# PaddlePaddle/Anakin

Hardware: AMD Instinct MI355X
Metric: ResNet50 INT8 images/sec + p50 latency @ batch 1/8, 1×MI355X (higher is better)
Workload: dtype int8

## Files before the change

### anakin_amd/csrc/api_chain.hip

```cpp
#include "api_internal.h"

enum : unsigned { CK_1X1 = 1, CK_3X3 = 2, CK_HEAD = 4, CK_PAIR = 8, CK_LED = CK_3X3 | CK_HEAD, CK_ANY = 15 };
static unsigned chain_kind(const saber_hip_chain* ch) { return !ch->c3 ? CK_1X1 : (ch->b2 ? CK_PAIR : (ch->b ? CK_3X3 : CK_HEAD)); }
static const struct { int c1; unsigned kinds; ChainForm f; } chain_forms[] = {
    {64, CK_ANY,            {4, 4, 4, 1, 1, CS_BASE, false}},
    {64, CK_ANY,            {2, 2, 4, 1, 1, CS_BASE, false}},
    {128, CK_1X1 | CK_LED,  {2, 2, 4, 1, 1, CS_BASE, false}},
    {128, CK_1X1 | CK_LED,  {1, 1, 4, 1, 1, CS_BASE, false}},
    {128, CK_1X1 | CK_LED,  {6, 2, 8, 1, 1, CS_W8, false}},
    {128, CK_1X1 | CK_LED,  {5, 1, 8, 1, 1, CS_W8, false}},
    {256, CK_1X1 | CK_LED,  {1, 1, 4, 1, 1, CS_BASE, false}},
    {256, CK_1X1,           {9, 1, 4, 2, 1, CS_SPLIT, false}},
    {256, CK_1X1,           {11, 1, 8, 2, 1, CS_SPLIT8, false}},
    {256, CK_LED,           {3, 1, 8, 1, 1, CS_W8, false}},
    {256, CK_3X3,           {7, 1, 8, 1, 2, CS_COOP2, true}},
    {256, CK_3X3,           {15, 2, 8, 1, 4, CS_COOP4, true}},
    {512, CK_1X1,           {1, 1, 4, 1, 1, CS_BASE, false}},
    {512, CK_1X1,           {9, 1, 4, 2, 1, CS_SPLIT, false}},
};
static void for_each_chain_form(const saber_hip_chain* ch, const std::function<void(const ChainForm&)>& fn) {
    for (const auto& r : chain_forms)
        if (r.c1 == ch->c1 && (r.kinds & chain_kind(ch))) fn(r.f);
}
static ChainForm chain_form_where(const saber_hip_chain* ch, const std::function<bool(const ChainForm& row, const ChainForm& found)>& take) {
// ... 159 lines not shown
    hipError_t e = sp->d_w.upload(w);
    if (e == hipSuccess) e = sp->d_prm.upload(prm);
    if (e != hipSuccess) {
        delete sp;
        return hip_fail(e, "stem pair: device copies");
    }
    *out = sp;
    return SABER_HIP_OK;
}
void saber_hip_conv2d_stem_pair_destroy(saber_hip_stem_pair_t* sp) { delete sp; }
int saber_hip_conv2d_stem_pair_run(saber_hip_stem_pair_t* sp, const void* x, void* y_pool, void* y_a, void* y_b, void* workspace,
                                   saber_hip_stream_t stream) {
    if (g_capture) return capture_unsupported("saber_hip_conv2d_stem_pair_run (an executor-level object: saber_hip_net_optimize forms it itself)");
    if (!sp || !x || !y_a || !y_b) return fail(SABER_HIP_INVALID_VALUE, "null argument");
    saber_hip_conv* op = sp->stem;
    if (op->ws_bytes && !workspace) return fail(SABER_HIP_INVALID_VALUE, "workspace required");
    saber_mi355x::StemPairKArgs ka;
    const int rc = stem_pool_args(op, x, y_pool, workspace, (hipStream_t)stream, &ka.c);
    if (rc) return rc;
    ka.t.w = sp->d_w.p; ka.t.prm = sp->d_prm.p; ka.t.y1 = y_a; ka.t.y2 = y_b;
    ka.t.K1 = sp->a->d.k; ka.t.K2 = sp->b->d.k;
    ka.t.relu1 = sp->a->d.act == SABER_HIP_ACT_RELU; ka.t.relu2 = sp->b->d.act == SABER_HIP_ACT_RELU;
    ka.t.u8_1 = sp->a->d.out_dtype == SABER_HIP_U8; ka.t.u8_2 = sp->b->d.out_dtype == SABER_HIP_U8;
    HIP_TRY(saber_mi355x::launch_conv_stem_pool_pair(op->pre_quant ? 1 : 0, ka, (hipStream_t)stream));
    return SABER_HIP_OK;
}
saber_hip_chain::~saber_hip_chain() {
    if (h_coop_err) (void)hipHostFree(h_coop_err);
    delete stage1;
}
static unsigned div_magic(int d) { return d >= 2 ? (unsigned)((0x100000000ull + (unsigned)d - 1) / (unsigned)d) : 0u; }
static int stage_build(saber_hip_chain* const* chains, int n, bool per_image, saber_hip_chain* tail, saber_hip_chain_stage** out,
                       const saber_hip_conv* head_a = nullptr, const saber_hip_conv* head_b = nullptr) {
    if (!chains || n <= 0 || n > saber_mi355x::STAGE4_LONG || !out) return fail(SABER_HIP_INVALID_VALUE, "stage: 1..24 chains");
    if (head_a || head_b) {
        if (!head_a || !head_b) return fail(SABER_HIP_INVALID_VALUE, "null argument");
        if (!chains[0] || chains[0]->c1 != 256) return fail(SABER_HIP_INVALID_VALUE, "stage: a head goes with a C = 256 stage only");
        if (!per_image) return fail(SABER_HIP_INVALID_VALUE, "stage: a head needs an image per XCD");
        for (const saber_hip_conv* o : {head_a, head_b})
            if (o->d.res_mode != SABER_HIP_RES_NONE) return fail(SABER_HIP_INVALID_VALUE, "stage: the head's convs carry no residual");
        for (const saber_hip_conv* o : {head_a, head_b}) {
            const saber_hip_conv_desc& d = o->d;
            if (!o->is_i8 || !o->weights_set || o->algo != ALGO_IGEMM_I8 || o->epi != EPI_I8_CONV || o->pair_k2 || o->pool_fused || o->pool2 || o->gpool ||
                o->pre_quant || o->pre_pad || d.kh != 1 || d.kw != 1 || d.stride_h != 1 || d.stride_w != 1 || d.pad_h != 0 || d.pad_w != 0 || d.group != 1 ||
                o->c_eff != d.c || d.act_negative_slope != 0.f || d.in_layout != SABER_HIP_NHWC || d.out_layout != SABER_HIP_NHWC ||
                (d.out_dtype != SABER_HIP_S8 && d.out_dtype != SABER_HIP_U8))
                return fail(SABER_HIP_INVALID_VALUE, "stage: the head must be two plain 1x1 / stride 1 / pad 0 INT8 NHWC convs with weights set");
// ... 405 lines not shown
```

### anakin_amd/csrc/api_conv.hip

```cpp
#include "api_internal.h"

namespace saber_api {
thread_local std::string g_err;

void* zero_page() {
    static std::mutex mu;
    static void* pages[64] = {nullptr};
    int dev = 0;
    if (hipGetDevice(&dev) != hipSuccess || dev < 0 || dev >= 64) return nullptr;
    std::lock_guard<std::mutex> lock(mu);
    if (!pages[dev]) {
        void* p = nullptr;
        if (hipMalloc(&p, 256) != hipSuccess) return nullptr;
        if (hipMemset(p, 0, 256) != hipSuccess || hipStreamSynchronize(nullptr) != hipSuccess) {
            (void)hipFree(p);
            return nullptr;
        }
        pages[dev] = p;
    }
    return pages[dev];
}

}

// ... 608 lines not shown

int saber_hip_conv2d_run(saber_hip_conv_t* op, const void* x, void* y, const void* res, void* workspace,
                         saber_hip_stream_t stream) {
    if (g_capture) return capture_conv(op, x, y, res);
    if (!op || !x || !y) return fail(SABER_HIP_INVALID_VALUE, "null argument");
    if (!op->weights_set) return fail(SABER_HIP_INVALID_VALUE, "set_weights not called");
    if (op->ws_bytes && !workspace) return fail(SABER_HIP_INVALID_VALUE, "workspace required");
    if (op->d.res_mode == SABER_HIP_RES_ELTWISE && !res) return fail(SABER_HIP_INVALID_VALUE, "residual tensor required");
    if (op->pair_k2) return fail(SABER_HIP_INVALID_VALUE, "sibling pair: use saber_hip_conv2d_run_pair");
    hipStream_t s = (hipStream_t)stream;
    const saber_hip_conv_desc& d = op->d;
    const void* xin = x;
    if (op->gpool) return fail(SABER_HIP_INVALID_VALUE, "conv + fused global pooling: use saber_hip_conv2d_run_gpool");
    if (op->sel.fam == FAM_IMG1) return img_conv_run(op, x, y, res, nullptr, s);
    if (op->stem32) {
        HIP_TRY(launch_conv_stem_f32_pool_raw((const float*)x, op->d_wstem32.p, op->has_bias ? op->d_bias.p : nullptr, (float*)y, d.n, d.h, d.w, op->oh,
                                              op->ow, op->pool_oh, op->pool_ow, op->stem32 - 1, s));
        return SABER_HIP_OK;
    }
    if (op->pool_fused) {
        ConvKArgs a;
        const int rc = stem_pool_args(op, x, y, workspace, s, &a);
        if (rc) return rc;
        HIP_TRY(launch_conv_stem_pool(op->pre_quant ? 1 : 0, a, s));
        return SABER_HIP_OK;
    }
    if (op->sel.fam == FAM_STEM && op->pre_quant) {
        ConvKArgs a;
        fill_args(op, a, x, y, res);
        a.Cin = d.c;
        a.qinv = 1.f / op->in_scale;
        HIP_TRY(launch_conv_stem(1, a, s));
        return SABER_HIP_OK;
    }
    if (op->pre_quant) {
        HIP_TRY(launch_quantize_nchw_to_nhwc(d.n, d.c, d.h, d.w, op->c_eff, DT_S8, op->in_scale, (const float*)x,
                                             workspace, s));
        xin = workspace;
    } else if (op->pre_pad) {
        HIP_TRY(launch_pad_channels_i8((size_t)d.n * d.h * d.w, d.c, 4, x, workspace, s));
        xin = workspace;
    } else if (op->pre_transpose) {
        HIP_TRY(launch_transpose_nchw_to_nhwc_f32(d.n, d.c, d.h, d.w, op->c_eff, (const float*)x, (float*)workspace, s));
        xin = workspace;
    }
    ConvKArgs a;
    fill_args(op, a, xin, y, res);
// ... 107 lines not shown
```

### anakin_amd/csrc/api_internal.h

```cpp
#pragma once
#include "../../include/saber_hip.h"
#include "kernels.h"

#include <cmath>
#include <cstdio>
#include <algorithm>
#include <cstdlib>
#include <cstring>
#include <functional>
#include <memory>
#include <mutex>
#include <string>
#include <utility>
#include <type_traits>
#include <vector>

using namespace saber_mi355x;

namespace saber_api {

extern thread_local std::string g_err;
inline int fail(int code, const std::string& msg) {
    g_err = msg;
    return code;
// ... 87 lines not shown
inline ConvSel sel_halo(const ConvSel& base, int rows) { return sel_family(base, FAM_HALO, rows); }
inline ConvSel sel_img(const ConvSel& base, int nw, int ib, int rb) {
    ConvSel s = sel_family(base, FAM_IMG);
    s.img_nw = nw; s.img_ib = ib; s.img_rb = rb;
    return s;
}
inline ConvSel sel_img1(const ConvSel& base) { return sel_family(base, FAM_IMG1); }
inline ConvSel sel_fc_small(const ConvSel& base) { return sel_family(base, FAM_FC_SMALL); }
inline ConvSel sel_b3h(ConvSel base, int variant) { base.dma = 0; return sel_family(base, FAM_B3H, variant); }
inline ConvSel sel_pw(ConvSel base, int variant) { base.dma = 0; return sel_family(base, FAM_PW, variant); }
inline ConvSel sel_dw(const ConvSel& base, int form) { return sel_family(base, FAM_DW, form); }
inline ConvSel sel_group(const ConvSel& base, int form) { return sel_family(base, FAM_GROUP, form); }

}
using namespace saber_api;

struct saber_hip_conv {
    saber_hip_conv_desc d;
    int oh = 0, ow = 0;
    int algo = ALGO_DIRECT_I8;
    ConvSel sel;
    int pool_fused = 0, pool_oh = 0, pool_ow = 0;
    int pool2 = 0;
    int stem32 = 0;
    DevBuf<uint8_t> d_wstem32;
    std::vector<float> w_stem_host;
    DevBuf<uint8_t> d_w3h1, d_w3h2;
    DevBuf<uint8_t> d_wpw;
    DevBuf<uint8_t> d_wdw;
    DevBuf<uint8_t> d_wg;
    DevBuf<float> d_fcpart;
    DevBuf<unsigned> d_fcctr;
    DevBuf<float> d_wfc;
    int gpool = 0;
    struct saber_hip_stage* img_stage = nullptr;
    bool no_placement = false;
    int epi = EPI_I8_CONV;
    bool is_i8 = false;
    int x_dtype = DT_S8;
    int c_eff = 0;
    bool pre_quant = false;
    bool pre_pad = false;
    bool pre_transpose = false;
    size_t ws_bytes = 0;
    int Kg = 0, Kg_pad = 0, kw_pad = 0;
    float in_scale = 1.f, out_scale = 1.f;
// ... 362 lines not shown
```

### anakin_amd/csrc/api_net_autotune.hip

```cpp
#include "api_internal.h"

static saber_hip_conv* net_op_conv(saber_hip_net* net, int index) {
    if (index < 0 || index >= (int)net->ops.size()) return nullptr;
    NetOp& o = net->ops[index];
    if (o.kind == OP_CONV || o.kind == OP_CONV_PAIR) return o.conv;
    if (o.kind == OP_FC || o.kind == OP_FC_Q) return o.fc ? o.fc->conv : nullptr;
    return nullptr;
}
int saber_hip_net_get_choice(saber_hip_net_t* net, int index) {
    saber_hip_conv* c = net_op_conv(net, index);
    int choice = (c && !c->pool_fused && (c->algo <= ALGO_IGEMM_F32 || dw_ok(c) || group_ok(c))) ? saber_hip_conv2d_get_tile(c) : 0;
    if (!c) return choice;
    const NetOp& o = net->ops[index];
    if (o.chain) choice |= (1 << 28) | ((o.chain_on ? o.chain->form.code : 0) << 24);
    if (o.chain3) choice |= (1 << 29) | ((o.led_on ? o.chain3->form.code : 0) << 24);
    if (o.sep) choice |= (3 << 28) | ((o.sep_on ? o.sep->form : 0) << 24);
    if (o.ir) choice |= (int)0x80000000u | ((o.ir_on ? o.ir->form : 0) << 24);
    if (o.fire) choice |= (int)0x80000000u | ((o.fire_on ? o.fire->form : 0) << 24);
    if (o.stage && o.stage_on) choice |= 1 << 30;
    if (o.stage && o.stage_on && o.tail_on) choice |= (int)0x80000000u;
    if (o.head_of >= 0 && net->ops[o.head_of].stage_on && net->ops[o.head_of].head_on) choice |= 1 << 29;
    return choice;
}
int saber_hip_net_stage_blocks(const saber_hip_net_t* net, int index) {
    if (!net || index < 0 || index >= (int)net->ops.size()) return 0;
    const NetOp& o = net->ops[index];
    return o.stage ? (o.stage->c1 == 64 ? -o.stage_n : o.stage_n) : 0;
}
int saber_hip_net_stage_head(const saber_hip_net_t* net, int index) {
    if (!net || index < 1 || index >= (int)net->ops.size() || !net->ops[index].stage) return -1;
    return net->ops[index - 1].head_of == index ? index - 1 : -1;
}
int saber_hip_net_set_choice(saber_hip_net_t* net, int index, int choice) {
    saber_hip_conv* c = net_op_conv(net, index);
    const bool ir_bits = c && net->ops[index].ir && ((unsigned)choice >> 30) == 2u;
    const int ir_tn = (choice >> 24) & 15;
    if (ir_bits && ir_tn && !ir_form_valid(net->ops[index].ir, ir_tn)) return saber_hip_conv2d_ir_set_tile(net->ops[index].ir, ir_tn);
    const bool fire_bits = c && net->ops[index].fire && ((unsigned)choice >> 30) == 2u;
    if (fire_bits && ir_tn && !fire_form_valid(net->ops[index].fire, ir_tn)) return saber_hip_conv2d_fire_set_tile(net->ops[index].fire, ir_tn);
    if (fire_bits && !(choice & 0xffffff)) {
        net_set_fire(net, index, ir_tn);
        net_drop_graph(net);
        return SABER_HIP_OK;
    }
    if (ir_bits && !(choice & 0xffffff)) {
        net_set_ir(net, index, ir_tn);
        net_drop_graph(net);
        return SABER_HIP_OK;
    }
    if (!c || !choice || c->pool_fused || (c->algo > ALGO_IGEMM_F32 && !dw_ok(c) && !group_ok(c))) return SABER_HIP_OK;
    if (net->reproducible_fp32 && !c->is_i8) return SABER_HIP_OK;
    if (net->ops[index].kind == OP_CONV_PAIR && index > 0 && net->ops[index - 1].stem_pair) return SABER_HIP_OK;
    const int chain_bits = (choice >> 24) & 63;
    const bool stage_on = ((choice >> 30) & 1) && !net->shared_device;
    const bool tail_on = stage_on && (((unsigned)choice >> 31) & 1u);
    choice &= 0xffffff;
    if (net->shared_device && ((choice >> 16) & 0xff) == 11) choice &= ~(0xf << 12);
    NetOp& o = net->ops[index];
    saber_hip_chain* ch = index + 1 >= (int)net->ops.size() ? nullptr : ((o.chain3 && (chain_bits & 32)) ? o.chain3 : ((o.chain && (chain_bits & 16)) ? o.chain : nullptr));
    int tn = chain_bits & 15;
    if (ch && net->shared_device && chain_form(ch, tn).placement) tn = chain_form_plain(ch).code;
    if (ch && tn && !chain_form_valid(ch, tn)) return saber_hip_conv2d_chain_set_tile(ch, tn);
    const bool sep_bits = o.sep && (chain_bits & 48) == 48;
    if (sep_bits && tn && !sep_form_valid(o.sep, tn)) return saber_hip_conv2d_sep_set_tile(o.sep, tn);
    int rc = choice ? saber_hip_conv2d_set_tile(c, choice) : SABER_HIP_OK;
    if (rc) return rc;
    o.res_note.clear();
    o.stage_name_kept = false;
    if (ch && tn) (void)saber_hip_conv2d_chain_set_tile(ch, tn);
// ... 105 lines not shown
        if (o.kind == OP_CONV_PAIR) {
            int rc = saber_hip_conv2d_autotune_pair(o.conv, T(o.in), T(o.out), T(o.out2), stream, iters);
            if (rc) return rc;
            continue;
        }
        saber_hip_conv* c = o.kind == OP_CONV ? o.conv : ((o.kind == OP_FC || o.kind == OP_FC_Q) ? o.fc->conv : nullptr);
        if (!c) continue;
        const void* xin = T(o.in);
        if (o.kind == OP_FC && o.fc->pre_quant) {
            int rq = net_launch(net, o, (hipStream_t)stream);
            if (rq) return rq;
            xin = net->arena + net->ws_off;
        }
        int rc = saber_hip_conv2d_autotune(c, xin, T(o.out), T(o.in2), net->arena + net->ws_off, stream, iters);
        if (rc) return rc;
        o.res_note.clear();
    }
    net_resolve(net);
    const char* log_env = std::getenv("SABER_HIP_AUTOTUNE_LOG");
    const bool log_cands = g_cold && log_env && log_env[0] == '1';
    auto log_cand = [&](const saber_hip_conv* c, const std::string& name, float t) {
        if (log_cands) std::fprintf(stderr, "autotune [%dx%dx%d c%d k%d %dx%d] %-40s %8.2f us\n", c->d.n, c->d.h, c->d.w, c->d.c, c->d.k, c->d.kh, c->d.kw, name.c_str(), t);
    };
    for (size_t i = 0; i < net->ops.size(); ++i)
        if (net->ops[i].stage) net_set_stage(net, (int)i, false);
    for (size_t i = 0; i < net->ops.size(); ++i) {
        NetOp& A = net->ops[i];
        const int ia = (int)i;
        NetOp* H = (ia > 0 && net->ops[ia - 1].chain3) ? &net->ops[ia - 1] : nullptr;
        if (!A.chain && !H) continue;
        const int first = H ? ia - 1 : ia;
        const int last = (A.chain || (H && H->chain3->b2)) ? ia + 1 : ia;
        hipStream_t s = (hipStream_t)stream;
        auto run_all = [&]() -> int {
            int rc = 0;
            for (int k = first; k <= last; ++k) rc |= net_launch(net, net->ops[k], s);
            return rc;
        };
        auto timed = [&](float* t) { return time_enqueued(s, run_all, 20, t); };
        float best = 0.f;
        int best_mode = 0, best_tn = 0;
        net_set_chain_mode(net, ia, 0);
        int rc = timed(&best);
        if (rc) return rc;
        log_cand(A.conv, "separate", best);
        for (int mode = A.chain ? 1 : 2; mode <= (H ? 2 : 1); ++mode) {
// ... 146 lines not shown
```

### anakin_amd/csrc/api_select.hip

```cpp
#include "api_internal.h"

bool dw_ok(const saber_hip_conv* op) {
    const saber_hip_conv_desc& d = op->d;
    if (op->algo != ALGO_DIRECT_I8 && op->algo != ALGO_DIRECT_F32) return false;
    if (d.res_mode != SABER_HIP_RES_NONE || op->pre_quant || op->pre_pad || op->pre_transpose || d.out_layout != SABER_HIP_NHWC) return false;
    if (op->is_i8 && op->epi != EPI_I8_CONV) return false;
    return conv_dw3x3_ok(!op->is_i8, d.n, d.c, d.k, d.group, d.kh, d.kw, d.stride_h, d.stride_w, d.pad_h, d.pad_w, d.dil_h, d.dil_w, op->oh, op->ow);
}
bool group_ok(const saber_hip_conv* op) {
    const saber_hip_conv_desc& d = op->d;
    if (op->algo != ALGO_DIRECT_I8 || !op->is_i8 || op->epi != EPI_I8_CONV) return false;
    if (d.res_mode != SABER_HIP_RES_NONE || op->pre_quant || op->pre_pad || d.in_layout != SABER_HIP_NHWC || d.out_layout != SABER_HIP_NHWC) return false;
    if (d.in_dtype != SABER_HIP_S8 && d.in_dtype != SABER_HIP_U8) return false;
    return conv_group3x3_ok(d.n, d.c, d.k, d.group, d.kh, d.kw, d.stride_h, d.stride_w, d.pad_h, d.pad_w, d.dil_h, d.dil_w, op->oh, op->ow);
}
static bool pw_variant_ok(const saber_hip_conv* op, int variant) {
    if (!pw_eligible(op)) return false;
    if (variant == 0) return conv1x1_pw_ok(op->c_eff, op->d.k);
    int tm, p, dd, mb;
    return conv1x1_pwk_variant(variant, &tm, &p, &dd, &mb) && conv1x1_pwk_ok(op->d.n * op->d.h * op->d.w, op->c_eff, op->d.k) &&
           (op->c_eff >> 7) >= dd;
}
bool b3_tile_ok(const saber_hip_conv* op, int tile, int ks) {
    if (op->algo != ALGO_IGEMM_F32 || !op->d_w3.p || tile < 0 || tile >= TILE_COUNT_B3 || (ks != 1 && ks != 2)) return false;
// ... 166 lines not shown
    case 10: *out = sel_fc_small(cur); return SABER_HIP_OK;
    case 11: *out = sel_b3(cur, low, (ks & 15) ? (ks & 15) : 1, ks >> 4); return SABER_HIP_OK;
    case 12: *out = sel_img1(cur); return SABER_HIP_OK;
    case 13: *out = sel_b3h(cur, low); return SABER_HIP_OK;
    case 14: *out = sel_pw(cur, low); return SABER_HIP_OK;
    case 16:
        if (!dw_ok(op) || low > DW3X3_FORMS) return fail(SABER_HIP_INVALID_VALUE, sel_requirements(FAM_DW));
        *out = low ? sel_dw(cur, low) : sel_direct(cur);
        return SABER_HIP_OK;
    case 17:
        if (!group_ok(op) || low > G3X3_FORMS) return fail(SABER_HIP_INVALID_VALUE, sel_requirements(FAM_GROUP));
        *out = low ? sel_group(cur, low) : sel_direct(cur);
        return SABER_HIP_OK;
    default: return fail(SABER_HIP_INVALID_VALUE, "bad staging variant");
    }
}

int saber_hip_conv2d_set_tile(saber_hip_conv_t* op, int tile) {
    if (op->stem32) {
        if (((tile >> 16) & 0xff) != 15 || (tile & 0xff) > 3) return fail(SABER_HIP_INVALID_VALUE, "FP32 stem launch: (15 << 16) | 0..3");
        op->stem32 = 1 + (tile & 0xff);
        return SABER_HIP_OK;
    }
    if (op->pool_fused) return fail(SABER_HIP_INVALID_VALUE, "fused conv+pooling has a single kernel");
    ConvSel s;
    const int rc = sel_decode(op, tile, &s);
    return rc ? rc : sel_set(op, s);
}
int saber_hip_conv2d_get_tile(const saber_hip_conv_t* op) { return sel_encode(op); }

void sel_name(saber_hip_conv* op) {
    static const char* an[] = {"igemm_i8", "igemm_i8_c4", "igemm_f32", "direct_i8", "direct_f32"};
    const ConvSel& s = op->sel;
    const saber_hip_conv_desc& d = op->d;
    const char* sum = d.res_mode == SABER_HIP_RES_SUM_INPLACE ? "+sum" : "";
    int bmk = 0, bnp = 0;
    int tm = 0, thr = 0, depth = 0, wgs = 0;
    char buf[96];
    if (op->stem32) snprintf(buf, sizeof buf, "stem7x7s2_maxpool3x3s2_f32_bf16x3_nchw_in");
    else if (op->pool_fused) snprintf(buf, sizeof buf, "stem7x7s2_maxpool3x3s2_i8_4x8%s", op->pre_quant ? "_fusedquant" : "");
    else switch (s.fam) {
    case FAM_STEM: snprintf(buf, sizeof buf, "stem7x7s2_i8_8x16%s", op->pre_quant ? "_fusedquant" : ""); break;
    case FAM_FC_SMALL:
        snprintf(buf, sizeof buf, op->algo == ALGO_IGEMM_F32 ? ((op->d_fcpart.p && !op->d_wfc.p) ? "fc_f32_splitk_16xk4" : "fc_f32_small_16xk4") : "fc_i8_small_16xk4");
        break;
    case FAM_PW:
        if (s.variant) {
            (void)conv1x1_pwk_variant(s.variant, &tm, &bnp, &depth, &wgs);
            snprintf(buf, sizeof buf, "pw1x1_f32_bf16x3_ksplit4_%dch_%dpx_d%d%s%s", tm * 16, bnp * 16, depth, wgs > 1 ? "_2wg" : "", sum);
        } else snprintf(buf, sizeof buf, "pw1x1_f32_bf16x3_regs_c%d_%dch_per_wave%s", op->c_eff, op->c_eff == 64 ? 64 : 32, sum);
        break;
    case FAM_B3H:
        (void)conv3x3_b3h_variant(s.variant, &bmk, &bnp, &tm, &thr);
        if (s.variant >= 6) snprintf(buf, sizeof buf, "pw1x1_f32_bf16x3_%dch_%dpx_w%d", bmk, bnp * 16, thr / 64);
        else snprintf(buf, sizeof buf, "halo3x3_f32_bf16x3_%dch_%dx16_w%d%s", bmk, bnp, thr / 64, op->pool2 ? "+maxpool2x2" : "");
        break;
    case FAM_IMG1: snprintf(buf, sizeof buf, "imgres%dx%d_i8_%dch%s", d.kh, d.kw, 16 * ((d.k / 16 + 31) / 32), op->gpool ? "+gpool" : ""); break;
    case FAM_IMG: snprintf(buf, sizeof buf, "img3x3_i8_%dimg_x_%drows_k16_w%d", s.img_ib, s.img_rb, s.img_nw); break;
    case FAM_HALO: snprintf(buf, sizeof buf, "halo3x3_i8_%dx16", s.variant); break;
    case FAM_DW: snprintf(buf, sizeof buf, "dw3x3_%s_%s", op->is_i8 ? "i8" : "f32", conv_dw3x3_form_name(s.variant, !op->is_i8)); break;
    case FAM_GROUP: snprintf(buf, sizeof buf, "g3x3_i8_%s", conv_group3x3_form_name(s.variant)); break;
    case FAM_DIRECT: snprintf(buf, sizeof buf, "%s", an[op->algo]); break;
    case FAM_B3:
// ... 151 lines not shown
```

### anakin_amd/csrc/conv_stem.h

```cpp
#pragma once
#include "epilogue_pack.h"

namespace saber_mi355x {

typedef int v2i __attribute__((ext_vector_type(2)));
typedef unsigned short us2_ __attribute__((ext_vector_type(2)));
__device__ __forceinline__ unsigned pk_max_u16_(unsigned a, unsigned b) {
    const us2_ r = __builtin_elementwise_max(__builtin_bit_cast(us2_, a), __builtin_bit_cast(us2_, b));
    return __builtin_bit_cast(unsigned, r);
}

template <bool F32IN, int NPIX, int ICP>
__device__ __forceinline__ void stage_input_patch(const ConvKArgs& a, int n, int iy0, int ix0, unsigned xmask, int tid,
                                                  unsigned* lds_x) {
    constexpr int NIT = (NPIX + 255) / 256;
    float fv[NIT][4];
    unsigned pv[NIT];
    bool ok[NIT];
    const size_t plane = (size_t)a.H * a.W;
#pragma unroll
    for (int it = 0; it < NIT; ++it) {
        const int idx = tid + it * 256;
        const int r = idx / ICP, c = idx - r * ICP;
        const int iy = iy0 + r, ix = ix0 + c;
        ok[it] = idx < NPIX && iy >= 0 && iy < a.H && ix >= 0 && ix < a.W;
        pv[it] = 0;
#pragma unroll
        for (int ch = 0; ch < 4; ++ch) fv[it][ch] = 0.f;
        if (ok[it]) {
            if constexpr (F32IN) {
                const float* xp = (const float*)a.x + ((size_t)n * a.Cin * a.H + iy) * a.W + ix;
#pragma unroll
                for (int ch = 0; ch < 4; ++ch)
                    if (ch < a.Cin) fv[it][ch] = xp[ch * plane];
            } else {
                pv[it] = ((const unsigned*)a.x)[((size_t)n * a.H + iy) * a.W + ix];
            }
        }
    }
#pragma unroll
    for (int it = 0; it < NIT; ++it) {
        const int idx = tid + it * 256;
        unsigned pk = pv[it];
        if constexpr (F32IN) {
            if (ok[it]) {
#pragma unroll
                for (int ch = 0; ch < 4; ++ch) {
                    if (ch < a.Cin) {
                        float v = __fmul_rn(fv[it][ch], a.qinv);
                        v = truncf(v + copysignf(0x1.fffffep-2f, v));
                        v = v < -128.f ? -128.f : (v > 127.f ? 127.f : v);
                        pk |= ((unsigned)((int)v) & 0xffu) << (8 * ch);
                    }
                }
            }
        }
        if (idx < NPIX) lds_x[idx] = pk ^ xmask;
    }
}

template <int EK, bool F32IN>
__global__ __launch_bounds__(256) void conv_stem7x7s2_kernel(const ConvKArgs a) {
    constexpr int TH = 8, TW = 16;
    constexpr int IR = (TH - 1) * 2 + 7 + 1;
    constexpr int ICP = 40;
// ... 295 lines not shown
            const int g = (wave + 4 * i) >> 1;
            if (g >= tng) break;
            const int kb = g * 32 + fq * 8;
            const v4i* pc = lds_tp + (kb >> 2) * 3;
            const v4i z = {0, 0, 0, 0};
            const v4i c0 = mma_step(taf[i][0], bfr, pc[2]), c1 = mma_step(taf[i][1], bfr, pc[5]);
            const bool second = kb >= t.K1;
            const bool ou8 = second ? t.u8_2 : t.u8_1;
            const float lo = (second ? t.relu2 : t.relu1) ? 0.f : -3.0e38f;
            const float off = ou8 ? 0.f : 128.f;
            const unsigned xm = ou8 ? 0u : 0x80808080u;
            const unsigned w0 = chain_out_pack(c0, z, __builtin_bit_cast(v4f, pc[1]), __builtin_bit_cast(v4f, pc[0]), lo, off, xm);
            const unsigned w1 = chain_out_pack(c1, z, __builtin_bit_cast(v4f, pc[4]), __builtin_bit_cast(v4f, pc[3]), lo, off, xm);
            if (tok) {
                uint8_t* y = second ? (uint8_t*)t.y2 + tpix * t.K2 + (kb - t.K1) : (uint8_t*)t.y1 + tpix * t.K1 + kb;
                *(uint2*)y = make_uint2(w0, w1);
            }
        }
        SABER_TL(6);
    }
    SABER_TL_FLUSH();
}

template <bool F32IN>
__global__ __launch_bounds__(256, 4) void conv_stem_pool_kernel(const ConvKArgs a) {
    conv_stem_pool_body<F32IN, false>(a, StemPairTail{});
}
template <bool F32IN>
__global__ __launch_bounds__(256, 4) void conv_stem_pool_pair_kernel(const StemPairKArgs ka) {
    conv_stem_pool_body<F32IN, true>(ka.c, ka.t);
}

static hipError_t launch_conv_stem_pool_inst(int f32_in, const ConvKArgs& a, hipStream_t s) {
    ConvKArgs b = a;
    b.npx = a.N * ((a.pool_ow + 7) / 8) * ((a.pool_oh + 3) / 4);
    b.nky = (a.K + 63) / 64;
    b.mg_npx = magic_div(b.npx, (long long)b.npx * b.nky);
    dim3 grid(b.npx * b.nky), block(256);
    if (f32_in) hipLaunchKernelGGL((conv_stem_pool_kernel<true>), grid, block, 0, s, b);
    else hipLaunchKernelGGL((conv_stem_pool_kernel<false>), grid, block, 0, s, b);
    return hipGetLastError();
}
static hipError_t launch_conv_stem_pool_pair_inst(int f32_in, const StemPairKArgs& ka, hipStream_t s) {
    StemPairKArgs b = ka;
    b.c.npx = ka.c.N * ((ka.c.pool_ow + 7) / 8) * ((ka.c.pool_oh + 3) / 4);
    b.c.nky = 1;
    b.c.mg_npx = magic_div(b.c.npx, (long long)b.c.npx);
    dim3 grid(b.c.npx), block(256);
    if (f32_in) hipLaunchKernelGGL((conv_stem_pool_pair_kernel<true>), grid, block, 0, s, b);
    else hipLaunchKernelGGL((conv_stem_pool_pair_kernel<false>), grid, block, 0, s, b);
    return hipGetLastError();
}

}
```

### anakin_amd/csrc/kernels.h

```cpp
#pragma once
#include <hip/hip_runtime.h>
#include <stddef.h>
#include <stdint.h>

#ifdef SABER_TIMELINE
extern __device__ unsigned long long* saber_tl_buf;
#define SABER_TL_DECL unsigned long long tl_[16] = {0, 0, 0, 0, 0, 0, 0, 0, 0, 0, 0, 0, 0, 0, 0, 0}
#define SABER_TL(i) tl_[i] = wall_clock64()
#define SABER_TL_FLUSH()                                                                   \
    do {                                                                                   \
        if (threadIdx.x == 0 && saber_tl_buf)                                              \
            for (int i_ = 0; i_ < 16; ++i_) saber_tl_buf[(size_t)blockIdx.x * 16 + i_] = tl_[i_]; \
    } while (0)
#else
#define SABER_TL_DECL do { } while (0)
#define SABER_TL(i) do { } while (0)
#define SABER_TL_FLUSH() do { } while (0)
#endif

namespace saber_mi355x {

enum { DT_F32 = 0, DT_S8 = 1, DT_U8 = 2 };

enum {
// ... 205 lines not shown
bool conv3x3_img_feasible(int C, int OW, int OH, int N, int nw, int ib, int rb);
bool conv3x3_b3h_variant(int variant, int* bmk, int* th, int* tm, int* threads);
bool conv1x1_pw_ok(int c, int k);
hipError_t launch_conv1x1_pw(const ConvKArgs& a, hipStream_t s);
bool conv1x1_pwk_variant(int v, int* tm, int* p, int* d, int* minb);
bool conv1x1_pwk_ok(int m, int c, int k);
hipError_t launch_conv1x1_pwk(int variant, const ConvKArgs& a, hipStream_t s);
hipError_t launch_conv3x3_b3h(int variant, const ConvKArgs& a, hipStream_t s);
hipError_t launch_fc_i8_small(const ConvKArgs& a, hipStream_t s);
bool fc_i8_small_ok(int m, int c, int kg_pad);
hipError_t launch_fc_f32_small(const ConvKArgs& a, bool packed, hipStream_t s);
int fc_f32_packed_steps(int c);
bool fc_f32_small_ok(int m, int c, int kg_pad);
bool fc_i8_small_softmax_ok(int m, int c, int kg_pad, int k);
hipError_t launch_fc_i8_small_softmax(const ConvKArgs& a, float* prob, unsigned* ctr, hipStream_t s);
bool fc_f32_splitk_ok(int m, int c, int kg_pad, int k, bool softmax);
size_t fc_f32_splitk_part_floats(int c, int k);
size_t fc_f32_splitk_counters(int k);
hipError_t launch_fc_f32_splitk(const ConvKArgs& a, float* part, unsigned* ctr, float* prob, hipStream_t s);
bool gemm_f32_rows_ok(int m, int k);
hipError_t launch_gemm_f32_rows(int m, int n, int k, float alpha, const float* A, const float* B, float beta, float* C, const void* zero,
                                hipStream_t s);
hipError_t launch_conv_stem(int f32_in, const ConvKArgs& a, hipStream_t s);
hipError_t launch_conv_stem_pool(int f32_in, const ConvKArgs& a, hipStream_t s);
hipError_t launch_conv_stem_pool_pair(int f32_in, const StemPairKArgs& a, hipStream_t s);
hipError_t launch_conv_direct(int is_f32, const ConvKArgs& a, int group, hipStream_t s);
constexpr int DW3X3_FORMS = 2;
const char* conv_dw3x3_form_name(int form, bool f32);
bool conv_dw3x3_ok(bool f32, int n, int c, int k, int group, int kh, int kw, int stride_h, int stride_w, int pad_h, int pad_w, int dil_h,
                   int dil_w, int oh, int ow);
hipError_t launch_conv_dw3x3(int form, bool f32, const ConvKArgs& a, hipStream_t s);
constexpr int G3X3_FORMS = 1;
const char* conv_group3x3_form_name(int form);
int conv_group3x3_steps(int cg);
bool conv_group3x3_ok(int n, int c, int k, int group, int kh, int kw, int stride_h, int stride_w, int pad_h, int pad_w, int dil_h, int dil_w,
                      int oh, int ow);
hipError_t launch_conv_group3x3(int form, const ConvKArgs& a, int group, hipStream_t s);

struct SepKArgs {
    const void* x;
    const void* wdw;
    const float* dw_bias;
    const float* dw_scale;
    const void* wpw;
    const void* prm;
    void* y_dw;
    void* y_pw;
    int N, H, W, C, OH, OW, K;
// ... 117 lines not shown
```

### anakin_amd/csrc/stem_pool.hip

```cpp
#include "conv_stem.h"
namespace saber_mi355x {
hipError_t launch_conv_stem_pool(int f32_in, const ConvKArgs& a, hipStream_t s) { return launch_conv_stem_pool_inst(f32_in, a, s); }
hipError_t launch_conv_stem_pool_pair(int f32_in, const StemPairKArgs& a, hipStream_t s) { return launch_conv_stem_pool_pair_inst(f32_in, a, s); }
}
```

### anakin_amd/saber.py

```python
import ctypes as C

import numpy as np
import torch

from . import lib as L

_TORCH_DT = {L.F32: torch.float32, L.S8: torch.int8, L.U8: torch.uint8}


def _stream():
    return C.c_void_p(torch.cuda.current_stream().cuda_stream)


def _p(t):
    return None if t is None else C.c_void_p(t.data_ptr())


def _np_ptr(a):
    return None if a is None else a.ctypes.data_as(C.c_void_p)


def dtype_code(t):
    return {torch.float32: L.F32, torch.int8: L.S8, torch.uint8: L.U8}[t.dtype]

# ... 83 lines not shown
        return self

    def out_shape(self):
        d = self.desc
        oh, ow = self.out_hw
        return (d.n, oh, ow, d.k) if d.out_layout == L.NHWC else (d.n, d.k, oh, ow)

    def new_output(self):
        return torch.empty(self.out_shape(), dtype=_TORCH_DT[self.desc.out_dtype], device="cuda")

    def dispatch(self, x, y, res=None):
        L.check(L.load().saber_hip_conv2d_run(self.h, _p(x), _p(y), _p(res), _p(self.ws), _stream()))
        if getattr(self, "post_act", None) is not None:
            active, slope, coef = self.post_act
            activation(active, y, y, slope, coef)
        return y

    def algo(self):
        return L.load().saber_hip_conv2d_algo(self.h).decode()

    def set_tile(self, tile):
        L.check(L.load().saber_hip_conv2d_set_tile(self.h, tile))

    def set_global_pooling(self):
        L.check(L.load().saber_hip_conv2d_set_global_pooling(self.h))
        return self

    def dispatch_gpool(self, x, y, y_pool, res=None):
        L.check(L.load().saber_hip_conv2d_run_gpool(self.h, _p(x), _p(y), _p(res), _p(y_pool), _stream()))
        return y, y_pool

    def tile_id(self):
        return L.load().saber_hip_conv2d_get_tile(self.h) & 0xff

    def autotune(self, x, y, res=None, iters=5):
        L.check(L.load().saber_hip_conv2d_autotune(self.h, _p(x), _p(y), _p(res), _p(self.ws), _stream(), iters))

    def quantized_weights(self):
        d = self.desc
        wq = np.empty((d.k, d.c // d.group, d.kh, d.kw), np.int8)
        ws = np.empty(d.k, np.float32)
        L.check(L.load().saber_hip_conv2d_get_quantized_weights(self.h, _np_ptr(wq), _np_ptr(ws)))
        return wq, ws

    def __del__(self):
        try:
# ... 878 lines not shown
```

Measured before the change: 39740.

## Add larger-tile 512-thread stem conv+maxpool kernel forms selected by autotune

Adds two new variants of the fused 7x7 stem conv + 3x3 maxpool kernel (and its pair tail). They use 512 threads and larger pooling tiles (7x8 and 7x7 instead of 4x8), which cuts halo recomputation of the overlapping conv rows and amortizes the weight staging over more pixels. The net autotuner times each form per stem op and keeps a new one only if it beats the default by a small margin. The form also gets persisted through get/set_tile. Larger tiles mean fewer blocks at batch 1, so occupancy and parallelism drop in exchange for the reuse.

```diff
diff --git a/anakin_amd/csrc/api_chain.hip b/anakin_amd/csrc/api_chain.hip
--- a/anakin_amd/csrc/api_chain.hip
+++ b/anakin_amd/csrc/api_chain.hip
@@ -205,7 +205,7 @@
     ka.t.K1 = sp->a->d.k; ka.t.K2 = sp->b->d.k;
     ka.t.relu1 = sp->a->d.act == SABER_HIP_ACT_RELU; ka.t.relu2 = sp->b->d.act == SABER_HIP_ACT_RELU;
     ka.t.u8_1 = sp->a->d.out_dtype == SABER_HIP_U8; ka.t.u8_2 = sp->b->d.out_dtype == SABER_HIP_U8;
-    HIP_TRY(saber_mi355x::launch_conv_stem_pool_pair(op->pre_quant ? 1 : 0, ka, (hipStream_t)stream));
+    HIP_TRY(saber_mi355x::launch_conv_stem_pool_pair(op->pre_quant ? 1 : 0, ka, (hipStream_t)stream, op->stem_form));
     return SABER_HIP_OK;
 }
 saber_hip_chain::~saber_hip_chain() {
diff --git a/anakin_amd/csrc/api_conv.hip b/anakin_amd/csrc/api_conv.hip
--- a/anakin_amd/csrc/api_conv.hip
+++ b/anakin_amd/csrc/api_conv.hip
@@ -654,7 +654,7 @@
         ConvKArgs a;
         const int rc = stem_pool_args(op, x, y, workspace, s, &a);
         if (rc) return rc;
-        HIP_TRY(launch_conv_stem_pool(op->pre_quant ? 1 : 0, a, s));
+        HIP_TRY(launch_conv_stem_pool(op->pre_quant ? 1 : 0, a, s, op->stem_form));
         return SABER_HIP_OK;
     }
     if (op->sel.fam == FAM_STEM && op->pre_quant) {
diff --git a/anakin_amd/csrc/api_internal.h b/anakin_amd/csrc/api_internal.h
--- a/anakin_amd/csrc/api_internal.h
+++ b/anakin_amd/csrc/api_internal.h
@@ -133,6 +133,7 @@
     ConvSel sel;
     int pool_fused = 0, pool_oh = 0, pool_ow = 0;
     int pool2 = 0;
+    int stem_form = 0;
     int stem32 = 0;
     DevBuf<uint8_t> d_wstem32;
     std::vector<float> w_stem_host;
diff --git a/anakin_amd/csrc/api_net_autotune.hip b/anakin_amd/csrc/api_net_autotune.hip
--- a/anakin_amd/csrc/api_net_autotune.hip
+++ b/anakin_amd/csrc/api_net_autotune.hip
@@ -11,6 +11,7 @@
     saber_hip_conv* c = net_op_conv(net, index);
     int choice = (c && !c->pool_fused && (c->algo <= ALGO_IGEMM_F32 || dw_ok(c) || group_ok(c))) ? saber_hip_conv2d_get_tile(c) : 0;
     if (!c) return choice;
+    if (c->pool_fused && !c->stem32 && c->stem_form) choice = saber_hip_conv2d_get_tile(c);
     const NetOp& o = net->ops[index];
     if (o.chain) choice |= (1 << 28) | ((o.chain_on ? o.chain->form.code : 0) << 24);
     if (o.chain3) choice |= (1 << 29) | ((o.led_on ? o.chain3->form.code : 0) << 24);
@@ -45,6 +46,13 @@
     }
     if (ir_bits && !(choice & 0xffffff)) {
         net_set_ir(net, index, ir_tn);
+        net_drop_graph(net);
+        return SABER_HIP_OK;
+    }
+    if (c && c->pool_fused && !c->stem32 && ((choice >> 16) & 0xff) == 18) {
+        const int rc = saber_hip_conv2d_set_tile(c, choice);
+        if (rc) return rc;
+        net_resolve(net);
         net_drop_graph(net);
         return SABER_HIP_OK;
     }
@@ -196,6 +204,29 @@
     auto log_cand = [&](const saber_hip_conv* c, const std::string& name, float t) {
         if (log_cands) std::fprintf(stderr, "autotune [%dx%dx%d c%d k%d %dx%d] %-40s %8.2f us\n", c->d.n, c->d.h, c->d.w, c->d.c, c->d.k, c->d.kh, c->d.kw, name.c_str(), t);
     };
+    for (size_t i = 0; i < net->ops.size(); ++i) {
+        NetOp& S = net->ops[i];
+        saber_hip_conv* c = S.kind == OP_CONV ? S.conv : nullptr;
+        if (!c || !c->pool_fused || c->stem32 || S.launch == LAUNCH_NONE) continue;
+        hipStream_t s = (hipStream_t)stream;
+        auto run_all = [&]() -> int { return net_launch(net, S, s); };
+        auto timed = [&](float* t) { return time_enqueued(s, run_all, 20, t); };
+        float best = 0.f;
+        int best_form = 0;
+        for (int form = 0; form < saber_mi355x::conv_stem_pool_form_count(); ++form) {
+            float us = -1.f;
+            if (saber_hip_conv2d_set_tile(c, (18 << 16) | form) != SABER_HIP_OK) continue;
+            const int rt = timed(&us);
+            if (form == 0 && rt) return rt;
+            log_cand(c, c->algo_name + (S.stem_pair ? "+pair" : ""), rt == SABER_HIP_OK ? us : -1.f);
+            if (form == 0) best = us;
+            else if (rt == SABER_HIP_OK && us < (best_form ? best : best * 0.99f)) { best = us; best_form = form; }
+        }
+        (void)saber_hip_conv2d_set_tile(c, (18 << 16) | best_form);
+        net_resolve(net);
+        const int rc = run_all();
+        if (rc) return rc;
+    }
     for (size_t i = 0; i < net->ops.size(); ++i)
         if (net->ops[i].stage) net_set_stage(net, (int)i, false);
     for (size_t i = 0; i < net->ops.size(); ++i) {
diff --git a/anakin_amd/csrc/api_select.hip b/anakin_amd/csrc/api_select.hip
--- a/anakin_amd/csrc/api_select.hip
+++ b/anakin_amd/csrc/api_select.hip
@@ -212,12 +212,21 @@
         op->stem32 = 1 + (tile & 0xff);
         return SABER_HIP_OK;
     }
-    if (op->pool_fused) return fail(SABER_HIP_INVALID_VALUE, "fused conv+pooling has a single kernel");
+    if (op->pool_fused) {
+        if (((tile >> 16) & 0xff) != 18 || (tile & 0xffff) >= conv_stem_pool_form_count() || (tile >> 24))
+            return fail(SABER_HIP_INVALID_VALUE, "fused conv+pooling: (18 << 16) | 0..2");
+        op->stem_form = tile & 0xff;
+        sel_name(op);
+        return SABER_HIP_OK;
+    }
     ConvSel s;
     const int rc = sel_decode(op, tile, &s);
     return rc ? rc : sel_set(op, s);
 }
-int saber_hip_conv2d_get_tile(const saber_hip_conv_t* op) { return sel_encode(op); }
+int saber_hip_conv2d_get_tile(const saber_hip_conv_t* op) {
+    if (op->pool_fused && !op->stem32) return (18 << 16) | op->stem_form;
+    return sel_encode(op);
+}
 
 void sel_name(saber_hip_conv* op) {
     static const char* an[] = {"igemm_i8", "igemm_i8_c4", "igemm_f32", "direct_i8", "direct_f32"};
@@ -228,7 +237,10 @@
     int tm = 0, thr = 0, depth = 0, wgs = 0;
     char buf[96];
     if (op->stem32) snprintf(buf, sizeof buf, "stem7x7s2_maxpool3x3s2_f32_bf16x3_nchw_in");
-    else if (op->pool_fused) snprintf(buf, sizeof buf, "stem7x7s2_maxpool3x3s2_i8_4x8%s", op->pre_quant ? "_fusedquant" : "");
+    else if (op->pool_fused) {
+        conv_stem_pool_form_dims(op->stem_form, &bmk, &bnp);
+        snprintf(buf, sizeof buf, "stem7x7s2_maxpool3x3s2_i8_%dx%d%s", bmk, bnp, op->pre_quant ? "_fusedquant" : "");
+    }
     else switch (s.fam) {
     case FAM_STEM: snprintf(buf, sizeof buf, "stem7x7s2_i8_8x16%s", op->pre_quant ? "_fusedquant" : ""); break;
     case FAM_FC_SMALL:
diff --git a/anakin_amd/csrc/conv_stem.h b/anakin_amd/csrc/conv_stem.h
--- a/anakin_amd/csrc/conv_stem.h
+++ b/anakin_amd/csrc/conv_stem.h
@@ -10,17 +10,17 @@
     return __builtin_bit_cast(unsigned, r);
 }
 
-template <bool F32IN, int NPIX, int ICP>
+template <bool F32IN, int NPIX, int ICP, int NT = 256>
 __device__ __forceinline__ void stage_input_patch(const ConvKArgs& a, int n, int iy0, int ix0, unsigned xmask, int tid,
                                                   unsigned* lds_x) {
-    constexpr int NIT = (NPIX + 255) / 256;
+    constexpr int NIT = (NPIX + NT - 1) / NT;
     float fv[NIT][4];
     unsigned pv[NIT];
     bool ok[NIT];
     const size_t plane = (size_t)a.H * a.W;
 #pragma unroll
     for (int it = 0; it < NIT; ++it) {
-        const int idx = tid + it * 256;
+        const int idx = tid + it * NT;
         const int r = idx / ICP, c = idx - r * ICP;
         const int iy = iy0 + r, ix = ix0 + c;
         ok[it] = idx < NPIX && iy >= 0 && iy < a.H && ix >= 0 && ix < a.W;
@@ -40,7 +40,7 @@
     }
 #pragma unroll
     for (int it = 0; it < NIT; ++it) {
-        const int idx = tid + it * 256;
+        const int idx = tid + it * NT;
         unsigned pk = pv[it];
         if constexpr (F32IN) {
             if (ok[it]) {
@@ -382,6 +382,217 @@
     SABER_TL_FLUSH();
 }
 
+constexpr int STEM_POOL_FORMS = 3;
+__host__ __device__ inline void stem_pool_form_tile(int form, int* ph, int* pw) {
+    *ph = form == 0 ? 4 : 7;
+    *pw = form == 2 ? 7 : 8;
+}
+__host__ __device__ inline int stem_w_src_chunk(int d) {
+    const int lrow = d >> 4, t = lrow >> 4;
+    const int r = (t >> 1) * 32 + ((lrow >> 2) & 3) * 8 + (t & 1) * 4 + (lrow & 3);
+    return r * 16 + ((d & 15) ^ (lrow & 15));
+}
+template <bool F32IN, bool TAIL, int PH, int PW>
+__device__ __forceinline__ void conv_stem_pool_form_body(const ConvKArgs& a, const StemPairTail& t) {
+    constexpr int CR = 2 * PH + 1, CC = 2 * PW + 1, NPX = CR * CC;
+    constexpr int NG = ((NPX + 15) / 16 + 3) & ~3, TN = NG / 4;
+    constexpr int IR = (CR - 1) * 2 + 7 + 1, ICP = (CC - 1) * 2 + 8;
+    constexpr int TM = 2, NV = 8, WCH = 64 * 16;
+    constexpr int NT = 512;
+    constexpr int NPP = PH * PW, NPG = (NPP + 15) / 16;
+    static_assert(NG % 4 == 0, "pixel groups split over four wave columns");
+    static_assert(NPP <= 64 && NPG == 4, "one pooling pass; the tail's unit mapping: a pixel group per wave of a half");
+    static_assert(NPG * 16 * 20 <= IR * ICP, "the pair's B operand reuses the patch");
+
+    __shared__ v4i lds_w[WCH];
+    __shared__ __attribute__((aligned(16))) unsigned lds_x[IR * ICP];
+    __shared__ uint2 lds_c[NG * 16 * 8];
+    constexpr int TPC = 256;
+    __shared__ v4i lds_tp[TAIL ? TPC : 1];
+    constexpr int MAXG = 10;
+    __shared__ v4i lds_ta[TAIL ? MAXG * 2 * 64 : 1];
+    SABER_TL_DECL;
+    SABER_TL(0);
+
+    const int tid = threadIdx.x, lane = tid & 63, wave = tid >> 6;
+    if constexpr (TAIL)
+        if (wave < 4) lds_dma16((const v4i*)t.prm + tid, lds_tp + wave * 64);
+    const int wm = wave >> 2, wn = wave & 3;
+    const int frow = lane & 15, fq = lane >> 4;
+
+    int ptile, tile_ky;
+    xcd_tile(a, ptile, tile_ky);
+    const int tiles_x = (a.pool_ow + PW - 1) / PW, tiles_y = (a.pool_oh + PH - 1) / PH;
+    const int per_img = tiles_x * tiles_y;
+    const int n = ptile / per_img;
+    const int trem = ptile - n * per_img;
+    const int py0 = (trem / tiles_x) * PH, px0 = (trem % tiles_x) * PW;
+    const int cy0 = py0 * 2, cx0 = px0 * 2;
+    const int k_base = tile_ky * 64;
+
+    const int kb = k_base + wm * 32 + fq * NV;
+    ChanParams<NV> cp;
+    load_chan_params<NV>(a, kb, cp);
+
+    const v4i* w16 = (const v4i*)a.w;
+    const int w_row_chunks = a.Kg_pad >> 4;
+#pragma unroll
+    for (int it = 0; it < WCH / NT; ++it) {
+        const int src = stem_w_src_chunk(tid + it * NT);
+        lds_dma16(w16 + (size_t)(k_base + (src >> 4)) * w_row_chunks + (src & 15), lds_w + it * NT + wave * 64);
+    }
+    const int iy0 = cy0 * 2 - a.pad_h, ix0 = cx0 * 2 - a.pad_w;
+    const unsigned xmask = a.in_u8 ? 0x80808080u : 0u;
+    SABER_TL(1);
+    stage_input_patch<F32IN, IR * ICP, ICP, NT>(a, n, iy0, ix0, xmask, tid, lds_x);
+    SABER_TL(2);
+    asm volatile("s_waitcnt vmcnt(0)" ::: "memory");
+    if constexpr (TAIL) {
+        const int nfr = (t.K1 + t.K2) >> 4;
+        for (int f = wave; f < nfr; f += 8) lds_dma16((const v4i*)t.w + f * 64 + lane, lds_ta + f * 64);
+    }
+    __syncthreads();
+
+    v4i acc[TM][TN];
+#pragma unroll
+    for (int i = 0; i < TM; ++i)
+#pragma unroll
+        for (int j = 0; j < TN; ++j) acc[i][j] = v4i{0, 0, 0, 0};
+    int a_idx[TM];
+#pragma unroll
+    for (int i = 0; i < TM; ++i) {
+        const int row = (wm * TM + i) * 16 + frow;
+        a_idx[i] = row * 16 + (fq ^ (row & 15));
+    }
+    int b_off[TN];
+    bool ok[TN];
+#pragma unroll
+    for (int j = 0; j < TN; ++j) {
+        const int q = (wn * TN + j) * 16 + frow;
+        const int qq = q < NPX ? q : NPX - 1;
+        const int r = qq / CC, c = qq - r * CC;
+        b_off[j] = (2 * r + (fq >> 1)) * ICP + 2 * c + 4 * (fq & 1);
+        ok[j] = q < NPX && cy0 + r < a.OH && cx0 + c < a.OW;
+    }
+#pragma unroll
+    for (int ks = 0; ks < 4; ++ks) {
+        v4i af[TM], bf[TN];
+#pragma unroll
+        for (int i = 0; i < TM; ++i) af[i] = lds_w[a_idx[i] ^ (ks << 2)];
+#pragma unroll
+        for (int j = 0; j < TN; ++j) {
+            const v2i* p = (const v2i*)&lds_x[b_off[j] + ks * 2 * ICP];
+            const v2i lo = p[0], hi = p[1];
+            bf[j] = v4i{lo.x, lo.y, hi.x, hi.y};
+        }
+#pragma unroll
+        for (int i = 0; i < TM; ++i)
+#pragma unroll
+            for (int j = 0; j < TN; ++j) acc[i][j] = mma_step(af[i], bf[j], acc[i][j]);
+    }
+
+    SABER_TL(3);
+    const bool u8 = a.out_dtype == DT_U8;
+    const float lo_clamp = a.relu ? 0.f : -3.0e38f;
+    const float off = u8 ? 0.f : 128.f;
+#pragma unroll
+    for (int j = 0; j < TN; ++j) {
+        const int q = (wn * TN + j) * 16 + frow;
+        unsigned pk[2] = {0u, 0u};
+        if (ok[j]) {
+#pragma unroll
+            for (int v = 0; v < 2; ++v) {
+                unsigned w = 0;
+                float dq[4];
+#pragma unroll
+                for (int t = 0; t < 4; t += 2) {
+                    v2f d2 = {(float)(acc[v][j][t] + cp.comp[v * 4 + t]), (float)(acc[v][j][t + 1] + cp.comp[v * 4 + t + 1])};
+                    d2 = d2 + v2f{cp.bias[v * 4 + t], cp.bias[v * 4 + t + 1]};
+                    d2 = d2 * v2f{cp.scale[v * 4 + t], cp.scale[v * 4 + t + 1]};
+                    dq[t] = d2.x;
+                    dq[t + 1] = d2.y;
+                }
+                if (u8) {
+#pragma unroll
+                    for (int t = 0; t < 4; ++t) w = __builtin_amdgcn_cvt_pk_u8_f32(rintf(dq[t]), t, w);
+                } else {
+#pragma unroll
+                    for (int t = 0; t < 4; ++t) w = __builtin_amdgcn_cvt_pk_u8_f32(fmaxf(rintf(dq[t]), lo_clamp) + off, t, w);
+                }
+                pk[v] = w;
+            }
+        }
+        lds_c[q * 8 + wm * 4 + fq] = make_uint2(pk[0], pk[1]);
+    }
+    __syncthreads();
+
+    SABER_TL(4);
+    {
+        const int pp = tid >> 3, cg = tid & 7;
+        const int ppy = pp / PW, ppx = pp - ppy * PW;
+        const int poy = py0 + ppy, pox = px0 + ppx;
+        const int kc = k_base + cg * 8;
+        if ((NPP == 64 || pp < NPP) && poy < a.pool_oh && pox < a.pool_ow && kc < a.K) {
+            unsigned ev[2] = {0, 0}, od[2] = {0, 0};
+#pragma unroll
+            for (int dy = 0; dy < 3; ++dy)
+#pragma unroll
+                for (int dx = 0; dx < 3; ++dx) {
+                    const uint2 v = lds_c[((2 * ppy + dy) * CC + 2 * ppx + dx) * 8 + cg];
+                    ev[0] = pk_max_u16_(ev[0], v.x & 0x00ff00ffu);
+                    od[0] = pk_max_u16_(od[0], (v.x >> 8) & 0x00ff00ffu);
+                    ev[1] = pk_max_u16_(ev[1], v.y & 0x00ff00ffu);
+                    od[1] = pk_max_u16_(od[1], (v.y >> 8) & 0x00ff00ffu);
+                }
+            const unsigned flip = u8 ? 0u : 0x80808080u;
+            const uint2 o = make_uint2((ev[0] | (od[0] << 8)) ^ flip, (ev[1] | (od[1] << 8)) ^ flip);
+            if constexpr (TAIL) {
+                *(uint2*)&lds_x[pp * 20 + cg * 2] = make_uint2(o.x ^ flip ^ 0x80808080u, o.y ^ flip ^ 0x80808080u);
+            }
+            if (!TAIL || a.y) {
+                uint8_t* y = (uint8_t*)a.y + (((size_t)n * a.pool_oh + poy) * a.pool_ow + pox) * a.K + kc;
+                if (kc + 8 <= a.K) *(uint2*)y = o;
+                else for (int t = 0; t < a.K - kc; ++t) y[t] = (uint8_t)((t < 4 ? o.x : o.y) >> (8 * (t & 3)));
+            }
+        }
+    }
+    SABER_TL(5);
+    if constexpr (TAIL) {
+        asm volatile("s_waitcnt vmcnt(0)" ::: "memory");
+        __syncthreads();
+        const int pg = wave & 3;
+        const v4i bfr = *(const v4i*)&lds_x[(pg * 16 + frow) * 20 + fq * 4];
+        const int tp = pg * 16 + frow;
+        const int toy = py0 + tp / PW, tox = px0 + tp % PW;
+        const bool tok = (NPP % 16 == 0 || tp < NPP) && toy < a.pool_oh && tox < a.pool_ow;
+        const size_t tpix = ((size_t)n * a.pool_oh + toy) * a.pool_ow + tox;
+        const int tng = (t.K1 + t.K2) >> 5;
+#pragma unroll
+        for (int u = 0; u < MAXG / 2; ++u) {
+            const int gu = (wave >> 2) + 2 * u;
+            const int g = gu < tng ? gu : tng - 1;
+            const int kb = g * 32 + fq * 8;
+            const v4i* pc = lds_tp + (kb >> 2) * 3;
+            const v4i z = {0, 0, 0, 0};
+            const v4i ta0 = lds_ta[(g * 2) * 64 + lane], ta1 = lds_ta[(g * 2 + 1) * 64 + lane];
+            const v4i c0 = mma_step(ta0, bfr, pc[2]), c1 = mma_step(ta1, bfr, pc[5]);
+            const bool second = kb >= t.K1;
+            const bool ou8 = second ? t.u8_2 : t.u8_1;
+            const float lo = (second ? t.relu2 : t.relu1) ? 0.f : -3.0e38f;
+            const float off = ou8 ? 0.f : 128.f;
+            const unsigned xm = ou8 ? 0u : 0x80808080u;
+            const unsigned w0 = chain_out_pack(c0, z, __builtin_bit_cast(v4f, pc[1]), __builtin_bit_cast(v4f, pc[0]), lo, off, xm);
+            const unsigned w1 = chain_out_pack(c1, z, __builtin_bit_cast(v4f, pc[4]), __builtin_bit_cast(v4f, pc[3]), lo, off, xm);
+            if (tok && gu < tng) {
+                uint8_t* y = second ? (uint8_t*)t.y2 + tpix * t.K2 + (kb - t.K1) : (uint8_t*)t.y1 + tpix * t.K1 + kb;
+                *(uint2*)y = make_uint2(w0, w1);
+            }
+        }
+        SABER_TL(6);
+    }
+    SABER_TL_FLUSH();
+}
+
 template <bool F32IN>
 __global__ __launch_bounds__(256, 4) void conv_stem_pool_kernel(const ConvKArgs a) {
     conv_stem_pool_body<F32IN, false>(a, StemPairTail{});
@@ -390,24 +601,50 @@
 __global__ __launch_bounds__(256, 4) void conv_stem_pool_pair_kernel(const StemPairKArgs ka) {
     conv_stem_pool_body<F32IN, true>(ka.c, ka.t);
 }
-
-static hipError_t launch_conv_stem_pool_inst(int f32_in, const ConvKArgs& a, hipStream_t s) {
+template <bool F32IN, int PH, int PW>
+__global__ __launch_bounds__(512, 2) void conv_stem_pool_form_kernel(const ConvKArgs a) {
+    conv_stem_pool_form_body<F32IN, false, PH, PW>(a, StemPairTail{});
+}
+template <bool F32IN, int PH, int PW>
+__global__ __launch_bounds__(512, 2) void conv_stem_pool_pair_form_kernel(const StemPairKArgs ka) {
+    conv_stem_pool_form_body<F32IN, true, PH, PW>(ka.c, ka.t);
+}
+
+static hipError_t launch_conv_stem_pool_inst(int f32_in, const ConvKArgs& a, hipStream_t s, int form) {
+    if (form < 0 || form >= STEM_POOL_FORMS) return hipErrorInvalidValue;
+    int ph, pw;
+    stem_pool_form_tile(form, &ph, &pw);
     ConvKArgs b = a;
-    b.npx = a.N * ((a.pool_ow + 7) / 8) * ((a.pool_oh + 3) / 4);
+    b.npx = a.N * ((a.pool_ow + pw - 1) / pw) * ((a.pool_oh + ph - 1) / ph);
     b.nky = (a.K + 63) / 64;
     b.mg_npx = magic_div(b.npx, (long long)b.npx * b.nky);
-    dim3 grid(b.npx * b.nky), block(256);
-    if (f32_in) hipLaunchKernelGGL((conv_stem_pool_kernel<true>), grid, block, 0, s, b);
+    dim3 grid(b.npx * b.nky), block(form ? 512 : 256);
+    if (form == 1) {
+        if (f32_in) hipLaunchKernelGGL((conv_stem_pool_form_kernel<true, 7, 8>), grid, block, 0, s, b);
+        else hipLaunchKernelGGL((conv_stem_pool_form_kernel<false, 7, 8>), grid, block, 0, s, b);
+    } else if (form == 2) {
+        if (f32_in) hipLaunchKernelGGL((conv_stem_pool_form_kernel<true, 7, 7>), grid, block, 0, s, b);
+        else hipLaunchKernelGGL((conv_stem_pool_form_kernel<false, 7, 7>), grid, block, 0, s, b);
+    } else if (f32_in) hipLaunchKernelGGL((conv_stem_pool_kernel<true>), grid, block, 0, s, b);
     else hipLaunchKernelGGL((conv_stem_pool_kernel<false>), grid, block, 0, s, b);
     return hipGetLastError();
 }
-static hipError_t launch_conv_stem_pool_pair_inst(int f32_in, const StemPairKArgs& ka, hipStream_t s) {
+static hipError_t launch_conv_stem_pool_pair_inst(int f32_in, const StemPairKArgs& ka, hipStream_t s, int form) {
+    if (form < 0 || form >= STEM_POOL_FORMS) return hipErrorInvalidValue;
+    int ph, pw;
+    stem_pool_form_tile(form, &ph, &pw);
     StemPairKArgs b = ka;
-    b.c.npx = ka.c.N * ((ka.c.pool_ow + 7) / 8) * ((ka.c.pool_oh + 3) / 4);
+    b.c.npx = ka.c.N * ((ka.c.pool_ow + pw - 1) / pw) * ((ka.c.pool_oh + ph - 1) / ph);
     b.c.nky = 1;
     b.c.mg_npx = magic_div(b.c.npx, (long long)b.c.npx);
-    dim3 grid(b.c.npx), block(256);
-    if (f32_in) hipLaunchKernelGGL((conv_stem_pool_pair_kernel<true>), grid, block, 0, s, b);
+    dim3 grid(b.c.npx), block(form ? 512 : 256);
+    if (form == 1) {
+        if (f32_in) hipLaunchKernelGGL((conv_stem_pool_pair_form_kernel<true, 7, 8>), grid, block, 0, s, b);
+        else hipLaunchKernelGGL((conv_stem_pool_pair_form_kernel<false, 7, 8>), grid, block, 0, s, b);
+    } else if (form == 2) {
+        if (f32_in) hipLaunchKernelGGL((conv_stem_pool_pair_form_kernel<true, 7, 7>), grid, block, 0, s, b);
+        else hipLaunchKernelGGL((conv_stem_pool_pair_form_kernel<false, 7, 7>), grid, block, 0, s, b);
+    } else if (f32_in) hipLaunchKernelGGL((conv_stem_pool_pair_kernel<true>), grid, block, 0, s, b);
     else hipLaunchKernelGGL((conv_stem_pool_pair_kernel<false>), grid, block, 0, s, b);
     return hipGetLastError();
 }
diff --git a/anakin_amd/csrc/kernels.h b/anakin_amd/csrc/kernels.h
--- a/anakin_amd/csrc/kernels.h
+++ b/anakin_amd/csrc/kernels.h
@@ -251,8 +251,11 @@
 hipError_t launch_gemm_f32_rows(int m, int n, int k, float alpha, const float* A, const float* B, float beta, float* C, const void* zero,
                                 hipStream_t s);
 hipError_t launch_conv_stem(int f32_in, const ConvKArgs& a, hipStream_t s);
-hipError_t launch_conv_stem_pool(int f32_in, const ConvKArgs& a, hipStream_t s);
-hipError_t launch_conv_stem_pool_pair(int f32_in, const StemPairKArgs& a, hipStream_t s);
+hipError_t launch_conv_stem_pool(int f32_in, const ConvKArgs& a, hipStream_t s, int form = 0);
+hipError_t launch_conv_stem_pool_pair(int f32_in, const StemPairKArgs& a, hipStream_t s, int form = 0);
+int conv_stem_pool_form_count();
+void conv_stem_pool_form_dims(int form, int* ph, int* pw);
+int conv_stem_w_src_chunk(int d);
 hipError_t launch_conv_direct(int is_f32, const ConvKArgs& a, int group, hipStream_t s);
 constexpr int DW3X3_FORMS = 2;
 const char* conv_dw3x3_form_name(int form, bool f32);
diff --git a/anakin_amd/csrc/stem_pool.hip b/anakin_amd/csrc/stem_pool.hip
--- a/anakin_amd/csrc/stem_pool.hip
+++ b/anakin_amd/csrc/stem_pool.hip
@@ -1,5 +1,8 @@
 #include "conv_stem.h"
 namespace saber_mi355x {
-hipError_t launch_conv_stem_pool(int f32_in, const ConvKArgs& a, hipStream_t s) { return launch_conv_stem_pool_inst(f32_in, a, s); }
-hipError_t launch_conv_stem_pool_pair(int f32_in, const StemPairKArgs& a, hipStream_t s) { return launch_conv_stem_pool_pair_inst(f32_in, a, s); }
+hipError_t launch_conv_stem_pool(int f32_in, const ConvKArgs& a, hipStream_t s, int form) { return launch_conv_stem_pool_inst(f32_in, a, s, form); }
+hipError_t launch_conv_stem_pool_pair(int f32_in, const StemPairKArgs& a, hipStream_t s, int form) { return launch_conv_stem_pool_pair_inst(f32_in, a, s, form); }
+int conv_stem_pool_form_count() { return STEM_POOL_FORMS; }
+void conv_stem_pool_form_dims(int form, int* ph, int* pw) { stem_pool_form_tile(form, ph, pw); }
+int conv_stem_w_src_chunk(int d) { return stem_w_src_chunk(d); }
 }
diff --git a/anakin_amd/saber.py b/anakin_amd/saber.py
--- a/anakin_amd/saber.py
+++ b/anakin_amd/saber.py
@@ -129,6 +129,9 @@
     def set_tile(self, tile):
         L.check(L.load().saber_hip_conv2d_set_tile(self.h, tile))
 
+    def get_tile(self):
+        return L.load().saber_hip_conv2d_get_tile(self.h)
+
     def set_global_pooling(self):
         L.check(L.load().saber_hip_conv2d_set_global_pooling(self.h))
         return self
```

Result: faster. 40140 (median of 6 runs) (+1.0%).
